# jkworldchampion/Video-Depth-Anything

Hardware: AMD Instinct MI355X
Metric: frames/sec at 1x32x518x518 fp16, ViT-L (higher is better)
Workload: dtype f16; 1 GPU; vitl fp16 32-frame clip forward, x=randn(1,32,3,518,518), seeded random weights (BASELINE.json configs[2]); parallelism=independent windows x1, world=1

## Files before the change

video_depth_anything_amd/csrc/host.hip:

```cpp
#include "vda_common.h"
#include <string.h>
#include <exception>
#include <type_traits>
#include <array>
#include <map>
#include <string>
#include <vector>

namespace {

constexpr int PATCH = 14, POS_GRID = 37, KPATCH = 640, GN_GROUPS = 32, TEMPORAL_HEADS = 8;
constexpr float ENC_LN_EPS = 1e-6f, GN_EPS = 1e-6f, TMP_LN_EPS = 1e-5f;

inline int pad64(int c) { return (c + 63) / 64 * 64; }

#define VDA_TRY(expr)            \
    do {                         \
        const int rc_ = (expr);  \
        if (rc_ != 0) return rc_; \
    } while (0)

#define VDA_HIP(expr)                                                      \
    do {                                                                   \
        const hipError_t e_ = (expr);                                      \
        if (e_ != hipSuccess) {                                            \
            vda_set_error("%s: %s", #expr, hipGetErrorString(e_));         \
            return 2;                                                      \
        }                                                                  \
// ... 65 lines not shown

struct Raw {
    float* d = nullptr;
    std::vector<int64_t> dims;
    size_t n = 0;
};

struct ProfSample {
    std::string name;
    double flops;
    hipEvent_t e0, e1;
};
struct Profile {
    int every = 0;
    double min_flops = 0.0;
    std::map<std::array<int, 5>, int> seen;
    std::map<std::string, std::pair<long long, double>> launches;
    std::vector<ProfSample> samples;
};

struct Layout {
    int gemm_launches = 0;
    std::map<std::string, std::pair<size_t, size_t>> bufs;
    std::vector<std::string> order;
    size_t total = 0;
};

}

struct vda_model {
    vda_config cfg;
    int device = 0;
    std::map<std::string, std::vector<int64_t>> spec;
    std::map<std::string, Raw> raw;
    std::map<std::string, void*> mat[2];
    std::map<std::string, float*> vec;
    bool finalized = false, packed[2] = {false, false};
    float oc3_bias = 0.f;
    void* zero_page = nullptr;
    std::map<std::pair<int, int>, float*> pos_cache;
    void* ws = nullptr;
    int64_t ws_bytes = 0;
    bool ws_owned = false;
    std::map<std::array<int, 5>, Layout> layouts;
    std::vector<void*> owned;
    int ocp[4] = {0, 0, 0, 0}, Fhp = 0;
    std::array<int, 5> last_key = {0, 0, 0, 0, -1};
    Profile prof;
    int residual_in_ln = 0;
    int dyn_sched = 0;
    int ln_fold = VDA_LN_FOLD_DEFAULT;
    int oc1_fused = 1;
    int head_overlap = 0;
    struct Side {
        hipStream_t stream = nullptr;
        hipEvent_t fork = nullptr, join = nullptr;
    };
    std::map<hipStream_t, Side> sides;
    int enc_split = 1;
    std::map<hipStream_t, Side> lanes;
    std::map<hipStream_t, hipEvent_t> tails;
    int mlp_fused = 0;
    volatile int32_t* ovf_host = nullptr;
};

namespace {

using Spec = std::map<std::string, std::vector<int64_t>>;

void build_spec(const vda_config& c, Spec& s) {
    const int64_t D = c.embed_dim, F = c.features;
    const int64_t oc[4] = {c.out_channels[0], c.out_channels[1], c.out_channels[2], c.out_channels[3]};
    auto put = [&](const std::string& k, std::vector<int64_t> v) { s[k] = std::move(v); };
    const std::string p = "pretrained.";
    put(p + "cls_token", {1, 1, D});
    put(p + "pos_embed", {1, POS_GRID * POS_GRID + 1, D});
    put(p + "mask_token", {1, D});
    put(p + "patch_embed.proj.weight", {D, 3, PATCH, PATCH});
    put(p + "patch_embed.proj.bias", {D});
    for (int i = 0; i < c.depth; ++i) {
        const std::string b = p + "blocks." + std::to_string(i) + ".";
        put(b + "norm1.weight", {D});
// ... 301 lines not shown
                h->vec[k + "ff1.b"] = (float*)bp;
                hipLaunchKernelGGL((pack_geglu_kernel<float>), dim3(grid_for((size_t)8 * Cc)), dim3(256), 0, s, raw(tb + "ff.net.0.proj.bias"), (float*)bp, 4 * Cc, 1);
            }
        }
        VDA_TRY(lin(k + "ff2.w", tb + "ff.net.2.weight", Cc, 4 * Cc, Cc, 4 * Cc));
        VDA_TRY(vecp(k + "ff2.b", tb + "ff.net.2.bias", Cc, Cc));
    }
    VDA_HIP(hipGetLastError());
    VDA_HIP(hipStreamSynchronize(s));
    h->packed[prec] = true;
    return 0;
}

struct Run {
    vda_model* h;
    int prec;
    bool dry;
    Layout* lay;
    hipStream_t s;
    size_t ab;
    int32_t* sched = nullptr;
    int nsched = 0;
    int mplan = 0;

    void* buf(const std::string& name, size_t elems, size_t esize) {
        const size_t bytes = (elems * esize + 255) & ~(size_t)255;
        if (dry) {
            auto it = lay->bufs.find(name);
            if (it == lay->bufs.end()) {
                lay->bufs[name] = {0, bytes};
                lay->order.push_back(name);
            } else if (it->second.second < bytes) {
                it->second.second = bytes;
            }
            return (void*)(uintptr_t)256;
        }
        return (char*)h->ws + lay->bufs.at(name).first;
    }
    void* act(const std::string& name, size_t elems) { return buf(name, elems, ab); }
    float* f32(const std::string& name, size_t elems) { return (float*)buf(name, elems, 4); }
    const void* W(const std::string& k) const { return dry ? nullptr : h->mat[prec].at(k); }
    const float* V(const std::string& k) const { return dry ? nullptr : h->vec.at(k); }

    int gemm(vda_gemm_args a) {
        if (prec == VDA_PREC_F16 && mplan == 0) {
            const int m1 = vda_gemm_plan_split(a.M, a.N, a.K, a.epilogue, a.a_mode);
            if (m1 < a.M) {
                if (dry) {
                    VDA_TRY(gemm_one(a));
                    return gemm_one(a);
                }
                vda_gemm_args p1, p2;
                a.zero_page = h->zero_page;
                VDA_TRY(vda_gemm_row_range(&a, 0, m1, &p1));
                VDA_TRY(vda_gemm_row_range(&a, m1, a.M - m1, &p2));
                p1.tile_rows = 256;
                p2.tile_rows = 192;
                VDA_TRY(gemm_one(p1));
                return gemm_one(p2);
            }
        }
        return gemm_one(a);
    }
    int gemm_one(vda_gemm_args a) {
        if (prec == VDA_PREC_F16 && h->dyn_sched) {
            if (!dry && sched != nullptr) a.sched = sched + 8 * nsched;
            ++nsched;
// ... 35 lines not shown
        return gemm(a);
    }
    int conv3x3(const void* x, const std::string& wname, void* out, int B, int H, int Wd, int Cin, int Cout, int epi, int stride,
                const float* bias, bool relu_in = false, const void* res = nullptr, const void* res2 = nullptr) {
        const int Ho = (H - 1) / stride + 1, Wo = (Wd - 1) / stride + 1;
        vda_gemm_args a = {};
        a.A = x, a.W = W(wname), a.out = out, a.bias = bias, a.res = res, a.res2 = res2;
        a.M = B * Ho * Wo, a.N = Cout, a.K = 9 * Cin, a.a_mode = VDA_A_CONV3X3, a.epilogue = epi, a.relu_in = relu_in ? 1 : 0;
        a.cB = B, a.cH = H, a.cW = Wd, a.cCin = Cin, a.cHo = Ho, a.cWo = Wo, a.cStride = stride;
        return gemm(a);
    }
    int layernorm(const float* x, void* out, const float* w, const float* b, float eps, int rows, int D, int group = 0, int skip = 0,
                  const float* pe = nullptr, int pe_rows = 0, int pe_steps = 0) {
        if (dry) return 0;
        return prec == VDA_PREC_F32 ? vda_layernorm_f32_f32(x, (float*)out, w, b, eps, rows, D, group, skip, pe, pe_rows, pe_steps, s)
                                    : vda_layernorm_f32_f16(x, out, w, b, eps, rows, D, group, skip, pe, pe_rows, pe_steps, s);
    }
    int bilinear(const void* x, void* out, int B, int hh, int ww, int H, int Wd, int C) {
        if (dry) return 0;
        return prec == VDA_PREC_F32 ? vda_bilinear_nhwc_f32((const float*)x, (float*)out, nullptr, B, hh, ww, H, Wd, C, s)
                                    : vda_bilinear_nhwc_f16(x, out, nullptr, B, hh, ww, H, Wd, C, s);
    }

    int temporal(int m, const void* x, int B, int T, int hw, int Cc, const std::string& tag, void** result) {
        const std::string k = "tm" + std::to_string(m) + ".";
        const int BT = B * T, rows = BT * hw;
        int chunks = (hw + 31) / 32;
        chunks = chunks < 1 ? 1 : (chunks > 16 ? 16 : chunks);
        float* part = f32("gn_partial", (size_t)BT * chunks * GN_GROUPS * 2);
        void* g = act("tm_g", (size_t)rows * Cc);
        if (!dry)
            VDA_TRY(prec == VDA_PREC_F32 ? vda_groupnorm_nhwc_f32((const float*)x, (float*)g, V(k + "gn.w"), V(k + "gn.b"), GN_EPS, BT, hw, Cc, GN_GROUPS, part, chunks, s)
                                         : vda_groupnorm_nhwc_f16(x, g, V(k + "gn.w"), V(k + "gn.b"), GN_EPS, BT, hw, Cc, GN_GROUPS, part, chunks, s));
        float* hs = f32("tm_hs", (size_t)rows * Cc);
        VDA_TRY(dense(g, W(k + "in.w"), hs, VDA_EPI_BIAS_F32, rows, Cc, Cc, V(k + "in.b")));
        void* n = act("tm_n", (size_t)rows * Cc);
        void* qkv = act("tm_qkv", (size_t)rows * 3 * Cc);
        void* ao = act("tm_ao", (size_t)rows * Cc);
        for (int a = 0; a < 2; ++a) {
            const std::string ka = k + "a" + std::to_string(a) + ".";
            const bool rope = h->cfg.pe_rope != 0;
            VDA_TRY(layernorm(hs, n, V(ka + "ln.w"), V(ka + "ln.b"), TMP_LN_EPS, rows, Cc, 0, 0, rope ? nullptr : V(ka + "pe"), hw, T));
            VDA_TRY(dense(n, W(ka + "qkv.w"), qkv, VDA_EPI_BIAS_F16, rows, 3 * Cc, Cc));
            for (int b = 0; b < B && !dry; ++b) {
                const size_t r0 = (size_t)b * T * hw;
                if (rope)
                    VDA_TRY(prec == VDA_PREC_F32 ? vda_rope_qk_f32((float*)qkv + r0 * 3 * Cc, T, hw, Cc, s) : vda_rope_qk_f16((h16*)qkv + r0 * 3 * Cc, T, hw, Cc, s));
                VDA_TRY(prec == VDA_PREC_F32
                            ? vda_temporal_attention_f32((const float*)qkv + r0 * 3 * Cc, (float*)ao + r0 * Cc, T, hw, Cc, TEMPORAL_HEADS, s)
                            : vda_temporal_attention_f16((const h16*)qkv + r0 * 3 * Cc, (h16*)ao + r0 * Cc, T, hw, Cc, TEMPORAL_HEADS, s));
            }
            VDA_TRY(dense(ao, W(ka + "out.w"), hs, VDA_EPI_SCALE_RES_F32, rows, Cc, Cc, V(ka + "out.b"), hs));
        }
        VDA_TRY(layernorm(hs, n, V(k + "ffln.w"), V(k + "ffln.b"), TMP_LN_EPS, rows, Cc));
        void* gg = act("tm_gg", (size_t)rows * 4 * Cc);
        VDA_TRY(dense(n, W(k + "ff1.w"), gg, VDA_EPI_GEGLU_F16, rows, 8 * Cc, Cc, V(k + "ff1.b"), nullptr, nullptr, 4 * Cc));
        void* hh = act("tm_hh", (size_t)rows * Cc);
        VDA_TRY(dense(gg, W(k + "ff2.w"), hh, VDA_EPI_SCALE_RES_F32_H, rows, Cc, 4 * Cc, V(k + "ff2.b"), hs));
        void* out = act(tag, (size_t)rows * Cc);
        VDA_TRY(dense(hh, W(k + "out.w"), out, VDA_EPI_RES_F16, rows, Cc, Cc, V(k + "out.b"), x));
        *result = out;
        return 0;
    }

    int rcu(int i, int u, const void* x, void* out, int B, int H, int Wd, int Fe, const void* res2 = nullptr) {
        const std::string k = "ref" + std::to_string(i) + ".rcu" + std::to_string(u) + ".";
        void* y = act("rcu_y", (size_t)B * H * Wd * Fe);
        VDA_TRY(conv3x3(x, k + "c1.w", y, B, H, Wd, Fe, Fe, VDA_EPI_BIAS_RELU_F16, 1, V(k + "c1.b"), true));
        VDA_TRY(conv3x3(y, k + "c2.w", out, B, H, Wd, Fe, Fe, VDA_EPI_RES_F16, 1, V(k + "c2.b"), false, x, res2));
        return 0;
    }
    int fusion(int i, const void* x0, const void* x1, int B, int H, int Wd, int Ho, int Wo, int Fe, const std::string& tag, void** result,
               bool upsample = true) {
        const size_t rows = (size_t)B * H * Wd;
        const void* sm = x0;
        if (x1 != nullptr) {
            void* t = act("fus_s", rows * Fe);
            VDA_TRY(rcu(i, 1, x1, t, B, H, Wd, Fe, x0));
            sm = t;
        }
        void* r = act("fus_r", rows * Fe);
        VDA_TRY(rcu(i, 2, sm, r, B, H, Wd, Fe));
        void* c = act(upsample ? "fus_c" : tag, rows * Fe);
        const std::string k = "ref" + std::to_string(i) + ".out.";
        VDA_TRY(dense(r, W(k + "w"), c, VDA_EPI_BIAS_F16, (int)rows, Fe, Fe, V(k + "b")));
        if (!upsample) {
            *result = c;
            return 0;
        }
        void* out = act(tag, (size_t)B * Ho * Wo * Fe);
        VDA_TRY(bilinear(c, out, B, H, Wd, Ho, Wo, Fe));
        *result = out;
        return 0;
    }

    int forward(const float* x, float* depth, int B, int T, int H, int Wd) {
        const vda_config& c = h->cfg;
        const int BT = B * T, ph = H / PATCH, pw = Wd / PATCH;
        const int P = ph * pw, D = c.embed_dim, NH = c.num_heads, Nt = P + 1, rows = BT * Nt;
        bool capturing = false;
        if (!dry) {
            hipStreamCaptureStatus cs = hipStreamCaptureStatusNone;
            if (hipStreamIsCapturing(s, &cs) != hipSuccess) {
                (void)hipGetLastError();
                cs = hipStreamCaptureStatusActive;
            }
            capturing = cs != hipStreamCaptureStatusNone;
        }
        if (prec == VDA_PREC_F16 && h->dyn_sched) {
            const int cap = dry ? 4096 : lay->gemm_launches;
            sched = (int32_t*)buf("sched", (size_t)8 * (cap > 0 ? cap : 1), 4);
            if (!dry) VDA_HIP(hipMemsetAsync(sched, 0, (size_t)32 * lay->gemm_launches, s));
            nsched = 0;
        }
// ... 8 lines not shown
            vda_gemm_args a = {};
            a.A = a0, a.W = W("patch.w"), a.out = tok, a.bias = V("patch.b"), a.pos = pos;
            a.M = BT * P, a.N = D, a.K = KPATCH, a.a_mode = VDA_A_DENSE, a.epilogue = VDA_EPI_PATCH_F32, a.P = P;
            VDA_TRY(gemm(a));
        }
        if (!dry) VDA_TRY(vda_cls_rows_f32(tok, V("cls"), pos, BT, P, D, s));
        void* xn = act("xn", (size_t)rows * D);
        void* qkv = act("qkv", (size_t)rows * 3 * D);
        void* ao = act("ao", (size_t)rows * D);
        void* hid = nullptr;
        void* taps[4] = {nullptr, nullptr, nullptr, nullptr};
        int ntap = 0;
        const bool defer = prec == VDA_PREC_F16 && h->residual_in_ln != 0;
        const bool fold = prec == VDA_PREC_F16 && h->ln_fold != 0 && !defer && D % 64 == 0;
        const bool mlp1 = fold && h->mlp_fused != 0 && vda_mlp_fused_supported(D, 4 * D) != 0;
        if (!mlp1) hid = act("hid", (size_t)rows * 4 * D);
        void* thi = fold ? buf("tok_hi", (size_t)rows * D, 2) : nullptr;
        void* tlo = fold ? buf("tok_lo", (size_t)rows * D, 2) : nullptr;
        float* lnpart = fold ? f32("ln_part", (size_t)rows * (D / 64) * 2) : nullptr;
        float* lnstat = fold ? f32("ln_stat", (size_t)rows * 2) : nullptr;
        int32_t* ovf = fold ? (int32_t*)buf("overflow", 1, 4) : nullptr;
        if (fold && !dry) VDA_HIP(hipMemsetAsync(ovf, 0, 4, s));
        if (fold && !dry) VDA_TRY(vda_split_center_stats_f32(tok, thi, tlo, lnstat, ENC_LN_EPS, rows, D, s));
        struct Part {
            int f0, nf;
            hipStream_t st;
        };
        Part parts[2] = {{0, BT, s}, {0, 0, nullptr}};
        int nparts = 1;
        vda_model::Side* lane = nullptr;
        bool split = fold && !mlp1 && h->enc_split != 0 && BT >= 2;
        if (split && !dry) {
            split = !capturing;
            for (auto& kv : h->tails) {
                if (!split) break;
                if (kv.first == s || kv.second == nullptr) continue;
                if (hipEventQuery(kv.second) != hipSuccess) {
                    (void)hipGetLastError();
                    split = false;
                }
            }
        }
        if (split) {
            parts[0] = {0, BT / 2, s};
            parts[1] = {BT / 2, BT - BT / 2, s};
            nparts = 2;
            if (!dry) {
                vda_model::Side& ln = h->lanes[s];
                if (ln.stream == nullptr) {
                    VDA_HIP(hipStreamCreateWithFlags(&ln.stream, hipStreamNonBlocking));
                    VDA_HIP(hipEventCreateWithFlags(&ln.fork, hipEventDisableTiming));
                    VDA_HIP(hipEventCreateWithFlags(&ln.join, hipEventDisableTiming));
                }
                lane = &ln;
                parts[1].st = ln.stream;
                VDA_HIP(hipEventRecord(ln.fork, s));
                VDA_HIP(hipStreamWaitEvent(ln.stream, ln.fork, 0));
            }
        }
        auto each = [&](auto&& fn) -> int {
            const hipStream_t keep = s;
            int rc = 0;
            for (int j = 0; j < nparts && rc == 0; ++j) {
                s = parts[j].st;
                rc = fn(parts[j]);
            }
            s = keep;
            return rc;
        };
        auto ln_gemm = [&](const std::string& wk, void* out, int epi, int N, const Part& p) -> int {
            const size_t r0 = (size_t)p.f0 * Nt;
            vda_gemm_args a = {};
            a.A = (const h16*)thi + r0 * D, a.W = W(wk + ".weight.ln"), a.out = (h16*)out + r0 * N, a.bias = V(wk + ".c2"), a.gamma = V(wk + ".c1");
            a.stats = lnstat + r0 * 2;
            a.M = p.nf * Nt, a.N = N, a.K = D, a.a_mode = VDA_A_DENSE, a.epilogue = epi;
            mplan = nparts > 1 ? rows : 0;
            const int rc = gemm(a);
            mplan = 0;
            return rc;
        };
        auto res_gemm = [&](const void* A, const std::string& wk, const std::string& gk, int K, bool stats_next, const Part& p) -> int {
// ... 11 lines not shown
            VDA_TRY(rc);
            (void)stats_next;
            if (!dry) VDA_TRY(vda_ln_stats_finalize(lnpart + r0 * np * 2, lnstat + r0 * 2, ENC_LN_EPS, nr, np, ovf, s));
            return 0;
        };
        auto tap_ln = [&](void* out, int group, int skip, const Part& p) -> int {
            if (dry) return 0;
            const size_t r0 = (size_t)p.f0 * Nt, o0 = group > 0 ? (size_t)p.f0 * (Nt / group) * (group - skip) : r0;
            const int nr = p.nf * Nt;
            return fold ? vda_layernorm_split_f16((const h16*)thi + r0 * D, (const h16*)tlo + r0 * D, (h16*)out + o0 * D, V("norm.w"), V("norm.b"), ENC_LN_EPS, nr, D,
                                                  group, skip, s)
                        : vda_layernorm_f32_f16(tok + r0 * D, (h16*)out + o0 * D, V("norm.w"), V("norm.b"), ENC_LN_EPS, nr, D, group, skip, nullptr, 0, 0, s);
        };
        void* yb = defer ? act("ybuf", (size_t)rows * D) : nullptr;
        auto ln_res = [&](const float* gamma, void* out, const float* w, const float* b, int group, int skip) -> int {
            if (dry) return 0;
            return vda_layernorm_residual_f32_f16(tok, yb, gamma, out, w, b, ENC_LN_EPS, rows, D, group, skip, s);
        };
        bool xn_ready = false;
        const int* ocp = h->ocp;
        const int Fe = c.features, Fhp = h->Fhp;
        const int h1 = 4 * ph, w1 = 4 * pw, h2 = 2 * ph, w2 = 2 * pw, h4 = (ph - 1) / 2 + 1, w4 = (pw - 1) / 2 + 1;
        void *l1r = nullptr, *l2r = nullptr, *l3r = nullptr;
        auto head_early = [&]() -> int {
            void* t0 = act("t0", (size_t)BT * P * ocp[0]);
            VDA_TRY(dense(taps[0], W("proj0.w"), t0, VDA_EPI_BIAS_F16, BT * P, ocp[0], D, V("proj0.b")));
            void* l1 = act("l1", (size_t)BT * h1 * w1 * ocp[0]);
            {
                vda_gemm_args a = {};
                a.A = t0, a.W = W("resize0.w"), a.out = l1, a.bias = V("resize0.b");
                a.M = BT * P, a.N = 16 * ocp[0], a.K = ocp[0], a.ldc = ocp[0], a.a_mode = VDA_A_DENSE, a.epilogue = VDA_EPI_CONVT_F16;
                a.tK = 4, a.tH = ph, a.tW = pw, a.tCout = ocp[0];
                VDA_TRY(gemm(a));
            }
            void* t1 = act("t1", (size_t)BT * P * ocp[1]);
            VDA_TRY(dense(taps[1], W("proj1.w"), t1, VDA_EPI_BIAS_F16, BT * P, ocp[1], D, V("proj1.b")));
            void* l2 = act("l2", (size_t)BT * h2 * w2 * ocp[1]);
            {
                vda_gemm_args a = {};
                a.A = t1, a.W = W("resize1.w"), a.out = l2, a.bias = V("resize1.b");
                a.M = BT * P, a.N = 4 * ocp[1], a.K = ocp[1], a.ldc = ocp[1], a.a_mode = VDA_A_DENSE, a.epilogue = VDA_EPI_CONVT_F16;
                a.tK = 2, a.tH = ph, a.tW = pw, a.tCout = ocp[1];
                VDA_TRY(gemm(a));
            }
            void* l3 = act("l3", (size_t)BT * P * ocp[2]);
            VDA_TRY(dense(taps[2], W("proj2.w"), l3, VDA_EPI_BIAS_F16, BT * P, ocp[2], D, V("proj2.b")));
            void* l3t = nullptr;
            VDA_TRY(temporal(0, l3, B, T, P, ocp[2], "l3t", &l3t));
            l1r = act("l1r", (size_t)BT * h1 * w1 * Fe);
            VDA_TRY(conv3x3(l1, "rn1.w", l1r, BT, h1, w1, ocp[0], Fe, VDA_EPI_BIAS_F16, 1, nullptr));
            l2r = act("l2r", (size_t)BT * h2 * w2 * Fe);
            VDA_TRY(conv3x3(l2, "rn2.w", l2r, BT, h2, w2, ocp[1], Fe, VDA_EPI_BIAS_F16, 1, nullptr));
            l3r = act("l3r", (size_t)BT * P * Fe);
            VDA_TRY(conv3x3(l3t, "rn3.w", l3r, BT, ph, pw, ocp[2], Fe, VDA_EPI_BIAS_F16, 1, nullptr));
            return 0;
        };
        bool early_done = false;
        vda_model::Side* side = nullptr;
        for (int i = 0; i < c.depth; ++i) {
            const std::string k = "b" + std::to_string(i) + ".";
            if (fold) {
                VDA_TRY(each([&](const Part& p) { return ln_gemm(k + "attn.qkv", qkv, VDA_EPI_LN_BIAS_F16, 3 * D, p); }));
            } else {
                if (!xn_ready) VDA_TRY(layernorm(tok, xn, V(k + "norm1.weight"), V(k + "norm1.bias"), ENC_LN_EPS, rows, D));
                xn_ready = false;
                VDA_TRY(dense(xn, W(k + "attn.qkv.weight"), qkv, VDA_EPI_BIAS_F16, rows, 3 * D, D, V(k + "attn.qkv.bias")));
            }
            if (!dry)
                VDA_TRY(each([&](const Part& p) {
                    const size_t r0 = (size_t)p.f0 * Nt;
                    return prec == VDA_PREC_F32 ? vda_attention_f32((const float*)qkv + r0 * 3 * D, (float*)ao + r0 * D, p.nf, Nt, NH, s)
                                                : vda_attention_f16((const h16*)qkv + r0 * 3 * D, (h16*)ao + r0 * D, p.nf, Nt, NH, s);
                }));
            if (fold) {
                VDA_TRY(each([&](const Part& p) { return res_gemm(ao, k + "attn.proj", k + "ls1.gamma", D, true, p); }));
            } else if (defer) {
                VDA_TRY(dense(ao, W(k + "attn.proj.weight"), yb, VDA_EPI_BIAS_F16, rows, D, D, V(k + "attn.proj.bias")));
                VDA_TRY(ln_res(V(k + "ls1.gamma"), xn, V(k + "norm2.weight"), V(k + "norm2.bias"), 0, 0));
// ... 62 lines not shown
                        if (sd.stream == nullptr) {
                            VDA_HIP(hipStreamCreateWithFlags(&sd.stream, hipStreamNonBlocking));
                            VDA_HIP(hipEventCreateWithFlags(&sd.fork, hipEventDisableTiming));
                            VDA_HIP(hipEventCreateWithFlags(&sd.join, hipEventDisableTiming));
                        }
                        side = &sd;
                        VDA_HIP(hipEventRecord(sd.fork, s));
                        VDA_HIP(hipStreamWaitEvent(sd.stream, sd.fork, 0));
                        if (lane != nullptr) {
                            VDA_HIP(hipEventRecord(lane->join, lane->stream));
                            VDA_HIP(hipStreamWaitEvent(sd.stream, lane->join, 0));
                        }
                        hipStream_t main_stream = s;
                        s = sd.stream;
                        const int rc = head_early();
                        s = main_stream;
                        if (rc != 0) return rc;
                        VDA_HIP(hipEventRecord(sd.join, sd.stream));
                        early_done = true;
                    }
                }
            }
        }
        if (lane != nullptr) {
            VDA_HIP(hipEventRecord(lane->join, lane->stream));
            VDA_HIP(hipStreamWaitEvent(s, lane->join, 0));
        }
        if (ntap != 4) {
            vda_set_error("vda_forward: the configuration's taps are not four distinct block indices below depth");
            return 1;
        }
        if (!early_done) VDA_TRY(head_early());
        else if (side != nullptr) VDA_HIP(hipStreamWaitEvent(s, side->join, 0));
        void* t3 = act("t3", (size_t)BT * P * ocp[3]);
        VDA_TRY(dense(taps[3], W("proj3.w"), t3, VDA_EPI_BIAS_F16, BT * P, ocp[3], D, V("proj3.b")));
        void* l4 = act("l4", (size_t)BT * h4 * w4 * ocp[3]);
        VDA_TRY(conv3x3(t3, "resize3.w", l4, BT, ph, pw, ocp[3], ocp[3], VDA_EPI_BIAS_F16, 2, V("resize3.b")));
        void* l4t = nullptr;
        VDA_TRY(temporal(1, l4, B, T, h4 * w4, ocp[3], "l4t", &l4t));
        void* l4r = act("l4r", (size_t)BT * h4 * w4 * Fe);
        VDA_TRY(conv3x3(l4t, "rn4.w", l4r, BT, h4, w4, ocp[3], Fe, VDA_EPI_BIAS_F16, 1, nullptr));
        void *p4 = nullptr, *p4t = nullptr, *p3 = nullptr, *p3t = nullptr, *p2 = nullptr, *p1 = nullptr;
        VDA_TRY(fusion(4, l4r, nullptr, BT, h4, w4, ph, pw, Fe, "p4", &p4));
        VDA_TRY(temporal(2, p4, B, T, P, Fe, "p4t", &p4t));
        VDA_TRY(fusion(3, p4t, l3r, BT, ph, pw, h2, w2, Fe, "p3", &p3));
        VDA_TRY(temporal(3, p3, B, T, h2 * w2, Fe, "p3t", &p3t));
        VDA_TRY(fusion(2, p3t, l2r, BT, h2, w2, h1, w1, Fe, "p2", &p2));
        const bool up_fused = prec == VDA_PREC_F16 && h->oc1_fused != 0 && Fhp <= 128 && Fe % 16 == 0;
        VDA_TRY(fusion(1, p2, l1r, BT, h1, w1, 2 * h1, 2 * w1, Fe, up_fused ? "p1c" : "p1", &p1, !up_fused));
        const int hh = 2 * h1, ww = 2 * w1;
        void* o1 = act("o1", (size_t)BT * hh * ww * Fhp);
        if (up_fused) {
            if (!dry) VDA_TRY(vda_conv3x3_up2_f16(p1, W("oc1.w"), V("oc1.b"), o1, BT, h1, w1, Fe, Fhp, Fhp, s));
        } else
            VDA_TRY(conv3x3(p1, "oc1.w", o1, BT, hh, ww, Fe, Fhp, VDA_EPI_BIAS_F16, 1, V("oc1.b")));
        if (prec == VDA_PREC_F16) {
            if (!dry) VDA_TRY(vda_depth_tail_f16(o1, W("oc2.w"), V("oc2.b"), V("oc3.w"), h->oc3_bias, depth, h->zero_page, BT, hh, ww, H, Wd, Fhp, s));
        } else {
            void* up = act("tail_up", (size_t)BT * H * Wd * Fhp);
            VDA_TRY(bilinear(o1, up, BT, hh, ww, H, Wd, Fhp));
            void* c2 = act("tail_c2", (size_t)BT * H * Wd * 32);
            VDA_TRY(conv3x3(up, "oc2.w", c2, BT, H, Wd, Fhp, 32, VDA_EPI_BIAS_RELU_F16, 1, V("oc2.b")));
            if (!dry) VDA_TRY(vda_head_out_f32_f32((const float*)c2, V("oc3.w"), h->oc3_bias, depth, (long long)BT * H * Wd, 32, s));
        }
        if (fold && !dry) {
            hipLaunchKernelGGL(poison_on_overflow_kernel, dim3(256), dim3(256), 0, s, (const int*)ovf, depth, (long long)BT * H * Wd, (volatile int*)h->ovf_host);
            VDA_LAUNCH_CHECK();
        }
        if (!dry && !capturing) {
            hipEvent_t& tail = h->tails[s];
            if (tail == nullptr) VDA_HIP(hipEventCreateWithFlags(&tail, hipEventDisableTiming));
            VDA_HIP(hipEventRecord(tail, s));
        }
        return 0;
    }
};

int get_layout(vda_model* h, int B, int T, int H, int W, int prec, Layout** out) {
    const std::array<int, 5> key = {B, T, H, W, prec};
    auto it = h->layouts.find(key);
    if (it == h->layouts.end()) {
        Layout lay;
        Run r{h, prec, true, &lay, nullptr, prec == VDA_PREC_F32 ? (size_t)4 : (size_t)2};
        VDA_TRY(r.forward(nullptr, nullptr, B, T, H, W));
        lay.gemm_launches = r.nsched;
        size_t off = 0;
        for (const std::string& n : lay.order) {
            lay.bufs[n].first = off;
            off += lay.bufs[n].second;
        }
        lay.total = off;
        it = h->layouts.emplace(key, std::move(lay)).first;
    }
    *out = &it->second;
    return 0;
}

int check_shape(const vda_model* h, int B, int T, int H, int W, int prec) {
    VDA_REQUIRE(prec == VDA_PREC_F16 || prec == VDA_PREC_F32, "vda_forward: precision %d (VDA_PREC_F16 = 0, VDA_PREC_F32 = 1)", prec);
    VDA_REQUIRE(B > 0 && T > 0, "vda_forward: empty clip B=%d T=%d", B, T);
    VDA_REQUIRE(H > 0 && H % PATCH == 0, "Input image height %d is not a multiple of patch height %d", H, PATCH);
    VDA_REQUIRE(W > 0 && W % PATCH == 0, "Input image width %d is not a multiple of patch width: %d", W, PATCH);
    VDA_REQUIRE(T <= h->cfg.num_frames, "vda_forward: T=%d exceeds temporal_max_len=%d", T, h->cfg.num_frames);
    VDA_REQUIRE((long long)B * T * ((H / PATCH) * (W / PATCH) + 1) * 4 * h->cfg.embed_dim < (1ll << 31), "vda_forward: clip too large for 32-bit row offsets (B*T*tokens*4*embed_dim)");
    return 0;
}

int enc_split_default() {
    static const int v = getenv("VDA_ENC_SPLIT") ? atoi(getenv("VDA_ENC_SPLIT")) : 1;
    return v != 0;
}

}

extern "C" int vda_create(const vda_config* cfg, vda_model** out) {
    VDA_REQUIRE(cfg && out, "vda_create: null argument");
    VDA_REQUIRE(cfg->embed_dim > 0 && cfg->embed_dim % 64 == 0 && cfg->num_heads > 0 && cfg->embed_dim == cfg->num_heads * 64,
                "vda_create: embed_dim=%d must be num_heads=%d x 64 (the attention kernels are built for head dim 64)", cfg->embed_dim, cfg->num_heads);
    VDA_REQUIRE(cfg->depth > 0 && cfg->features > 0 && cfg->features % 64 == 0, "vda_create: depth=%d features=%d (features must be a multiple of 64)", cfg->depth, cfg->features);
    VDA_REQUIRE(cfg->num_frames > 0 && cfg->num_frames <= 32, "vda_create: num_frames=%d must be in 1..32", cfg->num_frames);
    VDA_REQUIRE((cfg->use_clstoken | cfg->use_bn | cfg->pe_rope) >> 1 == 0, "vda_create: use_clstoken / use_bn / pe_rope are 0 or 1");
    for (int i = 0; i < 4; ++i) {
        VDA_REQUIRE(cfg->out_channels[i] > 0 && cfg->out_channels[i] % 8 == 0, "vda_create: out_channels[%d]=%d must be a positive multiple of 8", i, cfg->out_channels[i]);
        VDA_REQUIRE(cfg->taps[i] >= 0 && cfg->taps[i] < cfg->depth && (i == 0 || cfg->taps[i] > cfg->taps[i - 1]), "vda_create: taps must be increasing block indices below depth");
    }
    VDA_REQUIRE(cfg->out_channels[2] % 64 == 0 && cfg->out_channels[3] % 64 == 0,
                "vda_create: out_channels[2..3] carry the temporal modules (GroupNorm over the true width): multiples of 64 only");
    vda_model* h = new vda_model();
    h->cfg = *cfg;
    if (hipGetDevice(&h->device) != hipSuccess) {
        delete h;
        vda_set_error("vda_create: no HIP device (this library has no CPU path)");
        return 2;
    }
    for (int i = 0; i < 4; ++i) h->ocp[i] = pad64(cfg->out_channels[i]);
    h->Fhp = (cfg->features / 2 + 31) / 32 * 32;
    build_spec(h->cfg, h->spec);
    if (dev_alloc(h, 256, &h->zero_page) != 0 || hipMemset(h->zero_page, 0, 256) != hipSuccess) {
        for (void* p : h->owned) (void)hipFree(p);
        delete h;
        vda_set_error("vda_create: device allocation failed");
        return 2;
    }
    void* ring = nullptr;
    if (hipHostMalloc(&ring, 64, hipHostMallocDefault) != hipSuccess) {
        for (void* p : h->owned) (void)hipFree(p);
        delete h;
        vda_set_error("vda_create: pinned host allocation failed");
        return 2;
    }
    memset(ring, 0, 64);
    h->ovf_host = (volatile int32_t*)ring;
    h->enc_split = enc_split_default();
    *out = h;
    return 0;
}

extern "C" int vda_destroy(vda_model* h) {
    if (h == nullptr) return 0;
    if (h->ovf_host) (void)hipHostFree((void*)h->ovf_host);
    for (auto& kv : h->tails)
        if (kv.second) (void)hipEventDestroy(kv.second);
    for (auto* m : {&h->sides, &h->lanes})
        for (auto& kv : *m) {
            if (kv.second.fork) (void)hipEventDestroy(kv.second.fork);
            if (kv.second.join) (void)hipEventDestroy(kv.second.join);
            if (kv.second.stream) (void)hipStreamDestroy(kv.second.stream);
        }
    for (void* p : h->owned) (void)hipFree(p);
    delete h;
    return 0;
}

extern "C" int vda_num_weights(const vda_model* h) { return h ? (int)h->spec.size() : 0; }

static int vda_load_weight_impl(vda_model* h, const char* name, const void* ptr, const int64_t* dims, int ndim, int dtype) {
// ... 153 lines not shown
        h->layouts.clear();
        return 0;
    }
    if (strcmp(name, "profile_min_gflop") == 0) {
        h->prof.min_flops = 1e9 * value;
        return 0;
    }
    if (strcmp(name, "dyn_sched") == 0) {
        h->dyn_sched = value;
        h->layouts.clear();
        return 0;
    }
    if (strcmp(name, "ln_fold") == 0) {
        h->ln_fold = value;
        h->layouts.clear();
        return 0;
    }
    if (strcmp(name, "head_overlap") == 0) {
        h->head_overlap = value != 0;
        return 0;
    }
    if (strcmp(name, "enc_split") == 0) {
        h->enc_split = value < 0 ? enc_split_default() : value != 0;
        h->layouts.clear();
        return 0;
    }
    if (strcmp(name, "mlp_fused") == 0) {
        h->mlp_fused = value != 0;
        h->layouts.clear();
        return 0;
    }
    if (strcmp(name, "oc1_fused") == 0) {
        h->oc1_fused = value;
        h->layouts.clear();
        return 0;
    }
    vda_set_error("vda_set_option: unknown option %s", name);
    return 1;
}

extern "C" int vda_profile_start(vda_model* h, int every) {
    VDA_REQUIRE(h && every > 0, "vda_profile_start: bad arguments");
    VDA_REQUIRE(h->prof.samples.empty(), "vda_profile_start: a profile is already open");
    const double keep = h->prof.min_flops;
    h->prof = Profile();
    h->prof.every = every;
// ... 104 lines not shown
```

Measured before the change: 641.7 frames/s.

## Split DPT head into two frame halves on parallel streams with sync points

Extends the encoder's two-stream frame split into the depth head. Per-frame head stages (projections, convs, fusion blocks, temporal FFN, depth tail) are queued as steps and run on each half's stream with half-private scratch buffers. Streams only meet at the temporal attention, which needs all frames, and independent convs (rn1/rn2/rn3) are slotted in to fill those sync gaps. This targets idle time and the join barrier after the encoder, at the cost of more launches, smaller GEMMs, extra scratch memory and more complex event ordering.

```diff
diff --git a/video_depth_anything_amd/csrc/host.hip b/video_depth_anything_amd/csrc/host.hip
--- a/video_depth_anything_amd/csrc/host.hip
+++ b/video_depth_anything_amd/csrc/host.hip
@@ -4,6 +4,8 @@
 #include <type_traits>
 #include <array>
 #include <map>
+#include <algorithm>
+#include <functional>
 #include <string>
 #include <vector>
 
@@ -115,6 +117,7 @@
 struct Layout {
     int gemm_launches = 0;
     std::map<std::string, std::pair<size_t, size_t>> bufs;
+    std::map<std::string, size_t> hbase, hsize;
     std::vector<std::string> order;
     size_t total = 0;
 };
@@ -151,6 +154,7 @@
     };
     std::map<hipStream_t, Side> sides;
     int enc_split = 1;
+    int head_split = 1;
     std::map<hipStream_t, Side> lanes;
     std::map<hipStream_t, hipEvent_t> tails;
     int mlp_fused = 0;
@@ -498,6 +502,17 @@
     int32_t* sched = nullptr;
     int nsched = 0;
     int mplan = 0;
+    struct Part {
+        int f0, nf;
+        hipStream_t st;
+    };
+    Part hp[2] = {{0, 0, nullptr}, {0, 0, nullptr}};
+    int hn = 1;
+    int half = 0;
+    int fr_nf = 0, fr_bt = 0;
+    int horder = 0;
+    vda_model::Side* hlane = nullptr;
+    std::vector<std::function<int(const Part&)>> seg;
 
     void* buf(const std::string& name, size_t elems, size_t esize) {
         const size_t bytes = (elems * esize + 255) & ~(size_t)255;
@@ -515,10 +530,75 @@
     }
     void* act(const std::string& name, size_t elems) { return buf(name, elems, ab); }
     float* f32(const std::string& name, size_t elems) { return (float*)buf(name, elems, 4); }
+    void* hbuf(const std::string& name, size_t elems, size_t esize) {
+        char* p = (char*)buf(name, elems, esize);
+        if (dry) {
+            const size_t bytes = (elems * esize + 255) & ~(size_t)255;
+            size_t& m = (half == 0 ? lay->hbase : lay->hsize)[name];
+            if (m < bytes) m = bytes;
+            return p;
+        }
+        return half == 0 ? p : p + lay->hbase.at(name);
+    }
+    void* hact(const std::string& name, size_t elems) { return hbuf(name, elems, ab); }
+    const void* frame(const void* base, int f0, size_t per, size_t esize) const { return (const char*)base + (size_t)f0 * per * esize; }
+    void* frame(void* base, int f0, size_t per, size_t esize) const { return (char*)base + (size_t)f0 * per * esize; }
+
+    void step(std::function<int(const Part&)> fn) { seg.push_back(std::move(fn)); }
+    int on_part(int j, const std::function<int(const Part&)>& fn) {
+        const hipStream_t keep = s;
+        if (hn > 1) {
+            s = hp[j].st;
+            half = j;
+            fr_nf = hp[j].nf;
+        }
+        const int rc = fn(hp[j]);
+        s = keep;
+        half = 0;
+        fr_nf = 0;
+        return rc;
+    }
+    int flush() {
+        std::vector<std::function<int(const Part&)>> q;
+        q.swap(seg);
+        if (hn == 1 || horder == 0 || dry) {
+            for (const auto& fn : q)
+                for (int j = 0; j < hn; ++j) VDA_TRY(on_part(j, fn));
+            return 0;
+        }
+        const int a = horder == 2 ? 0 : 1, b = 1 - a;
+        for (const auto& fn : q) VDA_TRY(on_part(a, fn));
+        hipEvent_t ev = a == 0 ? hlane->fork : hlane->join;
+        VDA_HIP(hipEventRecord(ev, hp[a].st));
+        VDA_HIP(hipStreamWaitEvent(hp[b].st, ev, 0));
+        for (const auto& fn : q) VDA_TRY(on_part(b, fn));
+        return 0;
+    }
+    int meet(const std::function<int()>& fn, const std::function<int(const Part&)>& fill = nullptr) {
+        VDA_TRY(flush());
+        if (hn > 1 && !dry) {
+            VDA_HIP(hipEventRecord(hlane->join, hlane->stream));
+            VDA_HIP(hipStreamWaitEvent(s, hlane->join, 0));
+        }
+        if (fill && hn > 1) VDA_TRY(on_part(1, fill));
+        VDA_TRY(fn());
+        if (hn > 1 && !dry) {
+            VDA_HIP(hipEventRecord(hlane->fork, s));
+            VDA_HIP(hipStreamWaitEvent(hlane->stream, hlane->fork, 0));
+        }
+        if (fill) step([this, fill](const Part& p) -> int { return half == 0 ? fill(p) : 0; });
+        return 0;
+    }
     const void* W(const std::string& k) const { return dry ? nullptr : h->mat[prec].at(k); }
     const float* V(const std::string& k) const { return dry ? nullptr : h->vec.at(k); }
 
     int gemm(vda_gemm_args a) {
+        if (fr_nf != 0 && mplan == 0) {
+            mplan = a.M / fr_nf * fr_bt;
+            const int rc = gemm_one(a);
+            mplan = 0;
+            return rc;
+        }
         if (prec == VDA_PREC_F16 && mplan == 0) {
             const int m1 = vda_gemm_plan_split(a.M, a.N, a.K, a.epilogue, a.a_mode);
             if (m1 < a.M) {
@@ -600,74 +680,101 @@
                                     : vda_bilinear_nhwc_f16(x, out, nullptr, B, hh, ww, H, Wd, C, s);
     }
 
-    int temporal(int m, const void* x, int B, int T, int hw, int Cc, const std::string& tag, void** result) {
+    int temporal(int m, const void* x, int B, int T, int hw, int Cc, const std::string& tag, void** result,
+                 const std::function<int(const Part&)>* fills = nullptr) {
         const std::string k = "tm" + std::to_string(m) + ".";
-        const int BT = B * T, rows = BT * hw;
+        const int BT = B * T;
+        const size_t fe = (size_t)hw * Cc;
         int chunks = (hw + 31) / 32;
         chunks = chunks < 1 ? 1 : (chunks > 16 ? 16 : chunks);
-        float* part = f32("gn_partial", (size_t)BT * chunks * GN_GROUPS * 2);
-        void* g = act("tm_g", (size_t)rows * Cc);
-        if (!dry)
-            VDA_TRY(prec == VDA_PREC_F32 ? vda_groupnorm_nhwc_f32((const float*)x, (float*)g, V(k + "gn.w"), V(k + "gn.b"), GN_EPS, BT, hw, Cc, GN_GROUPS, part, chunks, s)
-                                         : vda_groupnorm_nhwc_f16(x, g, V(k + "gn.w"), V(k + "gn.b"), GN_EPS, BT, hw, Cc, GN_GROUPS, part, chunks, s));
-        float* hs = f32("tm_hs", (size_t)rows * Cc);
-        VDA_TRY(dense(g, W(k + "in.w"), hs, VDA_EPI_BIAS_F32, rows, Cc, Cc, V(k + "in.b")));
-        void* n = act("tm_n", (size_t)rows * Cc);
-        void* qkv = act("tm_qkv", (size_t)rows * 3 * Cc);
-        void* ao = act("tm_ao", (size_t)rows * Cc);
+        const bool rope = h->cfg.pe_rope != 0;
+        void* qkv = act("tm_qkv", (size_t)BT * 3 * fe);
+        void* ao = act("tm_ao", (size_t)BT * fe);
+        void* out = act(tag, (size_t)BT * fe);
+        auto ln_qkv = [=](const Part& p, int a) -> int {
+            const std::string ka = k + "a" + std::to_string(a) + ".";
+            const int rows = p.nf * hw;
+            const float* hs = (const float*)hbuf("tm_hs", (size_t)rows * Cc, 4);
+            void* n = hact("tm_n", (size_t)rows * Cc);
+            const float* pe = rope ? nullptr : V(ka + "pe");
+            const int lead = (pe == nullptr || p.f0 % T == 0) ? 0 : (p.nf < T - p.f0 % T ? p.nf : T - p.f0 % T);
+            if (lead > 0)
+                VDA_TRY(layernorm(hs, n, V(ka + "ln.w"), V(ka + "ln.b"), TMP_LN_EPS, lead * hw, Cc, 0, 0, pe + (size_t)(p.f0 % T) * Cc, hw, T));
+            if (lead < p.nf)
+                VDA_TRY(layernorm(hs + (size_t)lead * fe, frame(n, lead, fe, ab), V(ka + "ln.w"), V(ka + "ln.b"), TMP_LN_EPS, (p.nf - lead) * hw, Cc, 0, 0, pe,
+                                  hw, T));
+            return dense(n, W(ka + "qkv.w"), frame(qkv, p.f0, 3 * fe, ab), VDA_EPI_BIAS_F16, rows, 3 * Cc, Cc);
+        };
+        step([=](const Part& p) -> int {
+            const int rows = p.nf * hw;
+            float* part = (float*)hbuf("gn_partial", (size_t)p.nf * chunks * GN_GROUPS * 2, 4);
+            void* g = hact("tm_g", (size_t)rows * Cc);
+            const void* xp = frame(x, p.f0, fe, ab);
+            if (!dry)
+                VDA_TRY(prec == VDA_PREC_F32 ? vda_groupnorm_nhwc_f32((const float*)xp, (float*)g, V(k + "gn.w"), V(k + "gn.b"), GN_EPS, p.nf, hw, Cc, GN_GROUPS, part, chunks, s)
+                                             : vda_groupnorm_nhwc_f16(xp, g, V(k + "gn.w"), V(k + "gn.b"), GN_EPS, p.nf, hw, Cc, GN_GROUPS, part, chunks, s));
+            float* hs = (float*)hbuf("tm_hs", (size_t)rows * Cc, 4);
+            VDA_TRY(dense(g, W(k + "in.w"), hs, VDA_EPI_BIAS_F32, rows, Cc, Cc, V(k + "in.b")));
+            return ln_qkv(p, 0);
+        });
         for (int a = 0; a < 2; ++a) {
-            const std::string ka = k + "a" + std::to_string(a) + ".";
-            const bool rope = h->cfg.pe_rope != 0;
-            VDA_TRY(layernorm(hs, n, V(ka + "ln.w"), V(ka + "ln.b"), TMP_LN_EPS, rows, Cc, 0, 0, rope ? nullptr : V(ka + "pe"), hw, T));
-            VDA_TRY(dense(n, W(ka + "qkv.w"), qkv, VDA_EPI_BIAS_F16, rows, 3 * Cc, Cc));
-            for (int b = 0; b < B && !dry; ++b) {
-                const size_t r0 = (size_t)b * T * hw;
-                if (rope)
-                    VDA_TRY(prec == VDA_PREC_F32 ? vda_rope_qk_f32((float*)qkv + r0 * 3 * Cc, T, hw, Cc, s) : vda_rope_qk_f16((h16*)qkv + r0 * 3 * Cc, T, hw, Cc, s));
-                VDA_TRY(prec == VDA_PREC_F32
-                            ? vda_temporal_attention_f32((const float*)qkv + r0 * 3 * Cc, (float*)ao + r0 * Cc, T, hw, Cc, TEMPORAL_HEADS, s)
-                            : vda_temporal_attention_f16((const h16*)qkv + r0 * 3 * Cc, (h16*)ao + r0 * Cc, T, hw, Cc, TEMPORAL_HEADS, s));
-            }
-            VDA_TRY(dense(ao, W(ka + "out.w"), hs, VDA_EPI_SCALE_RES_F32, rows, Cc, Cc, V(ka + "out.b"), hs));
-        }
-        VDA_TRY(layernorm(hs, n, V(k + "ffln.w"), V(k + "ffln.b"), TMP_LN_EPS, rows, Cc));
-        void* gg = act("tm_gg", (size_t)rows * 4 * Cc);
-        VDA_TRY(dense(n, W(k + "ff1.w"), gg, VDA_EPI_GEGLU_F16, rows, 8 * Cc, Cc, V(k + "ff1.b"), nullptr, nullptr, 4 * Cc));
-        void* hh = act("tm_hh", (size_t)rows * Cc);
-        VDA_TRY(dense(gg, W(k + "ff2.w"), hh, VDA_EPI_SCALE_RES_F32_H, rows, Cc, 4 * Cc, V(k + "ff2.b"), hs));
-        void* out = act(tag, (size_t)rows * Cc);
-        VDA_TRY(dense(hh, W(k + "out.w"), out, VDA_EPI_RES_F16, rows, Cc, Cc, V(k + "out.b"), x));
+            VDA_TRY(meet([&]() -> int {
+                for (int b = 0; b < B && !dry; ++b) {
+                    const size_t r0 = (size_t)b * T * hw;
+                    if (rope)
+                        VDA_TRY(prec == VDA_PREC_F32 ? vda_rope_qk_f32((float*)qkv + r0 * 3 * Cc, T, hw, Cc, s) : vda_rope_qk_f16((h16*)qkv + r0 * 3 * Cc, T, hw, Cc, s));
+                    VDA_TRY(prec == VDA_PREC_F32
+                                ? vda_temporal_attention_f32((const float*)qkv + r0 * 3 * Cc, (float*)ao + r0 * Cc, T, hw, Cc, TEMPORAL_HEADS, s)
+                                : vda_temporal_attention_f16((const h16*)qkv + r0 * 3 * Cc, (h16*)ao + r0 * Cc, T, hw, Cc, TEMPORAL_HEADS, s));
+                }
+                return 0;
+            }, fills ? fills[a] : nullptr));
+            step([=](const Part& p) -> int {
+                const std::string ka = k + "a" + std::to_string(a) + ".";
+                const int rows = p.nf * hw;
+                float* hs = (float*)hbuf("tm_hs", (size_t)rows * Cc, 4);
+                VDA_TRY(dense(frame(ao, p.f0, fe, ab), W(ka + "out.w"), hs, VDA_EPI_SCALE_RES_F32, rows, Cc, Cc, V(ka + "out.b"), hs));
+                if (a == 0) return ln_qkv(p, 1);
+                void* n = hact("tm_n", (size_t)rows * Cc);
+                VDA_TRY(layernorm(hs, n, V(k + "ffln.w"), V(k + "ffln.b"), TMP_LN_EPS, rows, Cc));
+                void* gg = hact("tm_gg", (size_t)rows * 4 * Cc);
+                VDA_TRY(dense(n, W(k + "ff1.w"), gg, VDA_EPI_GEGLU_F16, rows, 8 * Cc, Cc, V(k + "ff1.b"), nullptr, nullptr, 4 * Cc));
+                void* hh = hact("tm_hh", (size_t)rows * Cc);
+                VDA_TRY(dense(gg, W(k + "ff2.w"), hh, VDA_EPI_SCALE_RES_F32_H, rows, Cc, 4 * Cc, V(k + "ff2.b"), hs));
+                return dense(hh, W(k + "out.w"), frame(out, p.f0, fe, ab), VDA_EPI_RES_F16, rows, Cc, Cc, V(k + "out.b"), frame(x, p.f0, fe, ab));
+            });
+        }
         *result = out;
         return 0;
     }
 
     int rcu(int i, int u, const void* x, void* out, int B, int H, int Wd, int Fe, const void* res2 = nullptr) {
         const std::string k = "ref" + std::to_string(i) + ".rcu" + std::to_string(u) + ".";
-        void* y = act("rcu_y", (size_t)B * H * Wd * Fe);
+        void* y = hact("rcu_y", (size_t)B * H * Wd * Fe);
         VDA_TRY(conv3x3(x, k + "c1.w", y, B, H, Wd, Fe, Fe, VDA_EPI_BIAS_RELU_F16, 1, V(k + "c1.b"), true));
         VDA_TRY(conv3x3(y, k + "c2.w", out, B, H, Wd, Fe, Fe, VDA_EPI_RES_F16, 1, V(k + "c2.b"), false, x, res2));
         return 0;
     }
     int fusion(int i, const void* x0, const void* x1, int B, int H, int Wd, int Ho, int Wo, int Fe, const std::string& tag, void** result,
                bool upsample = true) {
-        const size_t rows = (size_t)B * H * Wd;
-        const void* sm = x0;
-        if (x1 != nullptr) {
-            void* t = act("fus_s", rows * Fe);
-            VDA_TRY(rcu(i, 1, x1, t, B, H, Wd, Fe, x0));
-            sm = t;
-        }
-        void* r = act("fus_r", rows * Fe);
-        VDA_TRY(rcu(i, 2, sm, r, B, H, Wd, Fe));
-        void* c = act(upsample ? "fus_c" : tag, rows * Fe);
-        const std::string k = "ref" + std::to_string(i) + ".out.";
-        VDA_TRY(dense(r, W(k + "w"), c, VDA_EPI_BIAS_F16, (int)rows, Fe, Fe, V(k + "b")));
-        if (!upsample) {
-            *result = c;
-            return 0;
-        }
-        void* out = act(tag, (size_t)B * Ho * Wo * Fe);
-        VDA_TRY(bilinear(c, out, B, H, Wd, Ho, Wo, Fe));
+        const size_t fi = (size_t)H * Wd * Fe, fo = (size_t)Ho * Wo * Fe;
+        void* out = act(tag, (size_t)B * (upsample ? fo : fi));
+        step([=](const Part& p) -> int {
+            const size_t rows = (size_t)p.nf * H * Wd;
+            const void* x0p = frame(x0, p.f0, fi, ab);
+            const void* sm = x0p;
+            if (x1 != nullptr) {
+                void* t = hact("fus_s", rows * Fe);
+                VDA_TRY(rcu(i, 1, frame(x1, p.f0, fi, ab), t, p.nf, H, Wd, Fe, x0p));
+                sm = t;
+            }
+            void* r = hact("fus_r", rows * Fe);
+            VDA_TRY(rcu(i, 2, sm, r, p.nf, H, Wd, Fe));
+            void* c = upsample ? hact("fus_c", rows * Fe) : frame(out, p.f0, fi, ab);
+            const std::string k = "ref" + std::to_string(i) + ".out.";
+            VDA_TRY(dense(r, W(k + "w"), c, VDA_EPI_BIAS_F16, (int)rows, Fe, Fe, V(k + "b")));
+            return upsample ? bilinear(c, frame(out, p.f0, fo, ab), p.nf, H, Wd, Ho, Wo, Fe) : 0;
+        });
         *result = out;
         return 0;
     }
@@ -722,10 +829,6 @@
         int32_t* ovf = fold ? (int32_t*)buf("overflow", 1, 4) : nullptr;
         if (fold && !dry) VDA_HIP(hipMemsetAsync(ovf, 0, 4, s));
         if (fold && !dry) VDA_TRY(vda_split_center_stats_f32(tok, thi, tlo, lnstat, ENC_LN_EPS, rows, D, s));
-        struct Part {
-            int f0, nf;
-            hipStream_t st;
-        };
         Part parts[2] = {{0, BT, s}, {0, 0, nullptr}};
         int nparts = 1;
         vda_model::Side* lane = nullptr;
@@ -757,6 +860,16 @@
                 VDA_HIP(hipEventRecord(ln.fork, s));
                 VDA_HIP(hipStreamWaitEvent(ln.stream, ln.fork, 0));
             }
+        }
+        hp[0] = {0, BT, s};
+        hn = 1;
+        if (split && h->head_split != 0 && (dry || !h->head_overlap)) {
+            hp[0] = parts[0];
+            hp[1] = parts[1];
+            hn = 2;
+            fr_bt = BT;
+            hlane = lane;
+            horder = h->head_split == 2 || h->head_split == 3 ? h->head_split : 0;
         }
         auto each = [&](auto&& fn) -> int {
             const hipStream_t keep = s;
@@ -814,38 +927,58 @@
         const int Fe = c.features, Fhp = h->Fhp;
         const int h1 = 4 * ph, w1 = 4 * pw, h2 = 2 * ph, w2 = 2 * pw, h4 = (ph - 1) / 2 + 1, w4 = (pw - 1) / 2 + 1;
         void *l1r = nullptr, *l2r = nullptr, *l3r = nullptr;
+        std::function<int(const Part&)> rn3;
         auto head_early = [&]() -> int {
             void* t0 = act("t0", (size_t)BT * P * ocp[0]);
-            VDA_TRY(dense(taps[0], W("proj0.w"), t0, VDA_EPI_BIAS_F16, BT * P, ocp[0], D, V("proj0.b")));
             void* l1 = act("l1", (size_t)BT * h1 * w1 * ocp[0]);
-            {
-                vda_gemm_args a = {};
-                a.A = t0, a.W = W("resize0.w"), a.out = l1, a.bias = V("resize0.b");
-                a.M = BT * P, a.N = 16 * ocp[0], a.K = ocp[0], a.ldc = ocp[0], a.a_mode = VDA_A_DENSE, a.epilogue = VDA_EPI_CONVT_F16;
-                a.tK = 4, a.tH = ph, a.tW = pw, a.tCout = ocp[0];
-                VDA_TRY(gemm(a));
-            }
             void* t1 = act("t1", (size_t)BT * P * ocp[1]);
-            VDA_TRY(dense(taps[1], W("proj1.w"), t1, VDA_EPI_BIAS_F16, BT * P, ocp[1], D, V("proj1.b")));
             void* l2 = act("l2", (size_t)BT * h2 * w2 * ocp[1]);
-            {
-                vda_gemm_args a = {};
-                a.A = t1, a.W = W("resize1.w"), a.out = l2, a.bias = V("resize1.b");
-                a.M = BT * P, a.N = 4 * ocp[1], a.K = ocp[1], a.ldc = ocp[1], a.a_mode = VDA_A_DENSE, a.epilogue = VDA_EPI_CONVT_F16;
-                a.tK = 2, a.tH = ph, a.tW = pw, a.tCout = ocp[1];
-                VDA_TRY(gemm(a));
-            }
             void* l3 = act("l3", (size_t)BT * P * ocp[2]);
-            VDA_TRY(dense(taps[2], W("proj2.w"), l3, VDA_EPI_BIAS_F16, BT * P, ocp[2], D, V("proj2.b")));
+            void* const* tp = taps;
+            step([=](const Part& p) -> int {
+                const int m = p.nf * P;
+                VDA_TRY(dense(frame(tp[0], p.f0, (size_t)P * D, ab), W("proj0.w"), frame(t0, p.f0, (size_t)P * ocp[0], ab), VDA_EPI_BIAS_F16, m, ocp[0], D,
+                              V("proj0.b")));
+                {
+                    vda_gemm_args a = {};
+                    a.A = frame(t0, p.f0, (size_t)P * ocp[0], ab), a.W = W("resize0.w"), a.out = frame(l1, p.f0, (size_t)h1 * w1 * ocp[0], ab), a.bias = V("resize0.b");
+                    a.M = m, a.N = 16 * ocp[0], a.K = ocp[0], a.ldc = ocp[0], a.a_mode = VDA_A_DENSE, a.epilogue = VDA_EPI_CONVT_F16;
+                    a.tK = 4, a.tH = ph, a.tW = pw, a.tCout = ocp[0];
+                    VDA_TRY(gemm(a));
+                }
+                VDA_TRY(dense(frame(tp[1], p.f0, (size_t)P * D, ab), W("proj1.w"), frame(t1, p.f0, (size_t)P * ocp[1], ab), VDA_EPI_BIAS_F16, m, ocp[1], D,
+                              V("proj1.b")));
+                {
+                    vda_gemm_args a = {};
+                    a.A = frame(t1, p.f0, (size_t)P * ocp[1], ab), a.W = W("resize1.w"), a.out = frame(l2, p.f0, (size_t)h2 * w2 * ocp[1], ab), a.bias = V("resize1.b");
+                    a.M = m, a.N = 4 * ocp[1], a.K = ocp[1], a.ldc = ocp[1], a.a_mode = VDA_A_DENSE, a.epilogue = VDA_EPI_CONVT_F16;
+                    a.tK = 2, a.tH = ph, a.tW = pw, a.tCout = ocp[1];
+                    VDA_TRY(gemm(a));
+                }
+                return dense(frame(tp[2], p.f0, (size_t)P * D, ab), W("proj2.w"), frame(l3, p.f0, (size_t)P * ocp[2], ab), VDA_EPI_BIAS_F16, m, ocp[2], D,
+                             V("proj2.b"));
+            });
+            l1r = act("l1r", (size_t)BT * h1 * w1 * Fe);
+            l2r = act("l2r", (size_t)BT * h2 * w2 * Fe);
+            l3r = act("l3r", (size_t)BT * P * Fe);
+            void *o1r = l1r, *o2r = l2r, *o3r = l3r;
+            const std::function<int(const Part&)> fills[2] = {
+                [=](const Part& p) -> int {
+                    return conv3x3(frame(l1, p.f0, (size_t)h1 * w1 * ocp[0], ab), "rn1.w", frame(o1r, p.f0, (size_t)h1 * w1 * Fe, ab), p.nf, h1, w1, ocp[0], Fe,
+                                   VDA_EPI_BIAS_F16, 1, nullptr);
+                },
+                [=](const Part& p) -> int {
+                    return conv3x3(frame(l2, p.f0, (size_t)h2 * w2 * ocp[1], ab), "rn2.w", frame(o2r, p.f0, (size_t)h2 * w2 * Fe, ab), p.nf, h2, w2, ocp[1], Fe,
+                                   VDA_EPI_BIAS_F16, 1, nullptr);
+                }};
             void* l3t = nullptr;
-            VDA_TRY(temporal(0, l3, B, T, P, ocp[2], "l3t", &l3t));
-            l1r = act("l1r", (size_t)BT * h1 * w1 * Fe);
-            VDA_TRY(conv3x3(l1, "rn1.w", l1r, BT, h1, w1, ocp[0], Fe, VDA_EPI_BIAS_F16, 1, nullptr));
-            l2r = act("l2r", (size_t)BT * h2 * w2 * Fe);
-            VDA_TRY(conv3x3(l2, "rn2.w", l2r, BT, h2, w2, ocp[1], Fe, VDA_EPI_BIAS_F16, 1, nullptr));
-            l3r = act("l3r", (size_t)BT * P * Fe);
-            VDA_TRY(conv3x3(l3t, "rn3.w", l3r, BT, ph, pw, ocp[2], Fe, VDA_EPI_BIAS_F16, 1, nullptr));
-            return 0;
+            VDA_TRY(temporal(0, l3, B, T, P, ocp[2], "l3t", &l3t, fills));
+            rn3 = [=](const Part& p) -> int {
+                return conv3x3(frame(l3t, p.f0, (size_t)P * ocp[2], ab), "rn3.w", frame(o3r, p.f0, (size_t)P * Fe, ab), p.nf, ph, pw, ocp[2], Fe, VDA_EPI_BIAS_F16,
+                               1, nullptr);
+            };
+            if (hn == 1) step(rn3);
+            return flush();
         };
         bool early_done = false;
         vda_model::Side* side = nullptr;
@@ -954,7 +1087,7 @@
                 }
             }
         }
-        if (lane != nullptr) {
+        if (lane != nullptr && hn == 1) {
             VDA_HIP(hipEventRecord(lane->join, lane->stream));
             VDA_HIP(hipStreamWaitEvent(s, lane->join, 0));
         }
@@ -965,13 +1098,21 @@
         if (!early_done) VDA_TRY(head_early());
         else if (side != nullptr) VDA_HIP(hipStreamWaitEvent(s, side->join, 0));
         void* t3 = act("t3", (size_t)BT * P * ocp[3]);
-        VDA_TRY(dense(taps[3], W("proj3.w"), t3, VDA_EPI_BIAS_F16, BT * P, ocp[3], D, V("proj3.b")));
         void* l4 = act("l4", (size_t)BT * h4 * w4 * ocp[3]);
-        VDA_TRY(conv3x3(t3, "resize3.w", l4, BT, ph, pw, ocp[3], ocp[3], VDA_EPI_BIAS_F16, 2, V("resize3.b")));
+        step([=](const Part& p) -> int {
+            VDA_TRY(dense(frame(taps[3], p.f0, (size_t)P * D, ab), W("proj3.w"), frame(t3, p.f0, (size_t)P * ocp[3], ab), VDA_EPI_BIAS_F16, p.nf * P, ocp[3], D,
+                          V("proj3.b")));
+            return conv3x3(frame(t3, p.f0, (size_t)P * ocp[3], ab), "resize3.w", frame(l4, p.f0, (size_t)h4 * w4 * ocp[3], ab), p.nf, ph, pw, ocp[3], ocp[3],
+                           VDA_EPI_BIAS_F16, 2, V("resize3.b"));
+        });
         void* l4t = nullptr;
-        VDA_TRY(temporal(1, l4, B, T, h4 * w4, ocp[3], "l4t", &l4t));
+        const std::function<int(const Part&)> fills1[2] = {hn > 1 ? rn3 : nullptr, nullptr};
+        VDA_TRY(temporal(1, l4, B, T, h4 * w4, ocp[3], "l4t", &l4t, fills1));
         void* l4r = act("l4r", (size_t)BT * h4 * w4 * Fe);
-        VDA_TRY(conv3x3(l4t, "rn4.w", l4r, BT, h4, w4, ocp[3], Fe, VDA_EPI_BIAS_F16, 1, nullptr));
+        step([=](const Part& p) -> int {
+            return conv3x3(frame(l4t, p.f0, (size_t)h4 * w4 * ocp[3], ab), "rn4.w", frame(l4r, p.f0, (size_t)h4 * w4 * Fe, ab), p.nf, h4, w4, ocp[3], Fe,
+                           VDA_EPI_BIAS_F16, 1, nullptr);
+        });
         void *p4 = nullptr, *p4t = nullptr, *p3 = nullptr, *p3t = nullptr, *p2 = nullptr, *p1 = nullptr;
         VDA_TRY(fusion(4, l4r, nullptr, BT, h4, w4, ph, pw, Fe, "p4", &p4));
         VDA_TRY(temporal(2, p4, B, T, P, Fe, "p4t", &p4t));
@@ -982,18 +1123,31 @@
         VDA_TRY(fusion(1, p2, l1r, BT, h1, w1, 2 * h1, 2 * w1, Fe, up_fused ? "p1c" : "p1", &p1, !up_fused));
         const int hh = 2 * h1, ww = 2 * w1;
         void* o1 = act("o1", (size_t)BT * hh * ww * Fhp);
-        if (up_fused) {
-            if (!dry) VDA_TRY(vda_conv3x3_up2_f16(p1, W("oc1.w"), V("oc1.b"), o1, BT, h1, w1, Fe, Fhp, Fhp, s));
-        } else
-            VDA_TRY(conv3x3(p1, "oc1.w", o1, BT, hh, ww, Fe, Fhp, VDA_EPI_BIAS_F16, 1, V("oc1.b")));
-        if (prec == VDA_PREC_F16) {
-            if (!dry) VDA_TRY(vda_depth_tail_f16(o1, W("oc2.w"), V("oc2.b"), V("oc3.w"), h->oc3_bias, depth, h->zero_page, BT, hh, ww, H, Wd, Fhp, s));
-        } else {
-            void* up = act("tail_up", (size_t)BT * H * Wd * Fhp);
-            VDA_TRY(bilinear(o1, up, BT, hh, ww, H, Wd, Fhp));
-            void* c2 = act("tail_c2", (size_t)BT * H * Wd * 32);
-            VDA_TRY(conv3x3(up, "oc2.w", c2, BT, H, Wd, Fhp, 32, VDA_EPI_BIAS_RELU_F16, 1, V("oc2.b")));
-            if (!dry) VDA_TRY(vda_head_out_f32_f32((const float*)c2, V("oc3.w"), h->oc3_bias, depth, (long long)BT * H * Wd, 32, s));
+        void* up = prec == VDA_PREC_F16 ? nullptr : act("tail_up", (size_t)BT * H * Wd * Fhp);
+        void* c2 = prec == VDA_PREC_F16 ? nullptr : act("tail_c2", (size_t)BT * H * Wd * 32);
+        step([=](const Part& p) -> int {
+            const size_t pi = up_fused ? (size_t)h1 * w1 * Fe : (size_t)hh * ww * Fe;
+            const void* pp = frame(p1, p.f0, pi, ab);
+            void* op = frame(o1, p.f0, (size_t)hh * ww * Fhp, ab);
+            float* dp = dry ? nullptr : depth + (size_t)p.f0 * H * Wd;
+            if (up_fused) {
+                if (!dry) VDA_TRY(vda_conv3x3_up2_f16(pp, W("oc1.w"), V("oc1.b"), op, p.nf, h1, w1, Fe, Fhp, Fhp, s));
+            } else
+                VDA_TRY(conv3x3(pp, "oc1.w", op, p.nf, hh, ww, Fe, Fhp, VDA_EPI_BIAS_F16, 1, V("oc1.b")));
+            if (prec == VDA_PREC_F16) {
+                if (!dry) VDA_TRY(vda_depth_tail_f16(op, W("oc2.w"), V("oc2.b"), V("oc3.w"), h->oc3_bias, dp, h->zero_page, p.nf, hh, ww, H, Wd, Fhp, s));
+                return 0;
+            }
+            void* upp = frame(up, p.f0, (size_t)H * Wd * Fhp, ab);
+            void* c2p = frame(c2, p.f0, (size_t)H * Wd * 32, ab);
+            VDA_TRY(bilinear(op, upp, p.nf, hh, ww, H, Wd, Fhp));
+            VDA_TRY(conv3x3(upp, "oc2.w", c2p, p.nf, H, Wd, Fhp, 32, VDA_EPI_BIAS_RELU_F16, 1, V("oc2.b")));
+            return dry ? 0 : vda_head_out_f32_f32((const float*)c2p, V("oc3.w"), h->oc3_bias, dp, (long long)p.nf * H * Wd, 32, s);
+        });
+        VDA_TRY(flush());
+        if (hn > 1 && !dry) {
+            VDA_HIP(hipEventRecord(lane->join, lane->stream));
+            VDA_HIP(hipStreamWaitEvent(s, lane->join, 0));
         }
         if (fold && !dry) {
             hipLaunchKernelGGL(poison_on_overflow_kernel, dim3(256), dim3(256), 0, s, (const int*)ovf, depth, (long long)BT * H * Wd, (volatile int*)h->ovf_host);
@@ -1016,6 +1170,10 @@
         Run r{h, prec, true, &lay, nullptr, prec == VDA_PREC_F32 ? (size_t)4 : (size_t)2};
         VDA_TRY(r.forward(nullptr, nullptr, B, T, H, W));
         lay.gemm_launches = r.nsched;
+        for (const auto& kv : lay.hsize) {
+            size_t& bytes = lay.bufs.at(kv.first).second;
+            bytes = std::max(bytes, lay.hbase[kv.first] + kv.second);
+        }
         size_t off = 0;
         for (const std::string& n : lay.order) {
             lay.bufs[n].first = off;
@@ -1041,6 +1199,11 @@
 int enc_split_default() {
     static const int v = getenv("VDA_ENC_SPLIT") ? atoi(getenv("VDA_ENC_SPLIT")) : 1;
     return v != 0;
+}
+
+int head_split_default() {
+    static const int v = getenv("VDA_HEAD_SPLIT") ? atoi(getenv("VDA_HEAD_SPLIT")) : 1;
+    return v >= 0 && v <= 3 ? v : 1;
 }
 
 }
@@ -1084,6 +1247,7 @@
     memset(ring, 0, 64);
     h->ovf_host = (volatile int32_t*)ring;
     h->enc_split = enc_split_default();
+    h->head_split = head_split_default();
     *out = h;
     return 0;
 }
@@ -1283,6 +1447,12 @@
     }
     if (strcmp(name, "enc_split") == 0) {
         h->enc_split = value < 0 ? enc_split_default() : value != 0;
+        h->layouts.clear();
+        return 0;
+    }
+    if (strcmp(name, "head_split") == 0) {
+        VDA_REQUIRE(value <= 3, "vda_set_option: head_split is 0, 1, 2 or 3 (or < 0: the default)");
+        h->head_split = value < 0 ? head_split_default() : value;
         h->layouts.clear();
         return 0;
     }
```

New measurement: 648.4 frames/s, median of 6. +1.1%, better.
